# jesusdpa1/ssqueeze_rs

Hardware: NVIDIA B200
Metric: ssq_stft input Msamples/s (higher is better)
Workload: dtype f32

## Files before the change

ssqueeze_rs_b200/csrc/fft_regs.cuh:

```cuda
#pragma once
#include "stft_kernels.cuh"

template <bool PK = true>
__device__ __forceinline__ void fft8_fwd(float2 (&v)[8]) {
  const float S = 0.70710678118654752440f;
  float2 a0 = caddf<PK>(v[0], v[4]), a4 = csubf<PK>(v[0], v[4]);
  float2 a1 = caddf<PK>(v[1], v[5]), a5 = csubf<PK>(v[1], v[5]);
  float2 a2 = caddf<PK>(v[2], v[6]), a6 = csubf<PK>(v[2], v[6]);
  float2 a3 = caddf<PK>(v[3], v[7]), a7 = csubf<PK>(v[3], v[7]);
  float2 p5 = caddf<PK>(a5, cmi(a5));
  float2 p6 = cmi(a6);
  float2 p7 = csubf<PK>(cmi(a7), a7);
  float2 b0 = caddf<PK>(a0, a2), b2 = csubf<PK>(a0, a2);
  float2 b1 = caddf<PK>(a1, a3), b3 = csubf<PK>(a1, a3);
  float2 b4 = caddf<PK>(a4, p6), b6 = csubf<PK>(a4, p6);
  float2 b5 = caddf<PK>(p5, p7), b7 = csubf<PK>(p5, p7);
  float2 r3 = cmi(b3);
  float2 r7 = cmi(b7);
  v[0] = caddf<PK>(b0, b1);
  v[4] = csubf<PK>(b0, b1);
  v[2] = caddf<PK>(b2, r3);
  v[6] = csubf<PK>(b2, r3);
  v[1] = fma2<PK>(b5, bc2(S), b4);
  v[5] = fma2<PK>(b5, bc2(-S), b4);
  v[3] = fma2<PK>(r7, bc2(S), b6);
  v[7] = fma2<PK>(r7, bc2(-S), b6);
}

template <bool PK = true>
__device__ __forceinline__ void fft8_inv(float2 (&v)[8]) {
  const float S = 0.70710678118654752440f;
  float2 a0 = caddf<PK>(v[0], v[4]), a4 = csubf<PK>(v[0], v[4]);
  float2 a1 = caddf<PK>(v[1], v[5]), a5 = csubf<PK>(v[1], v[5]);
  float2 a2 = caddf<PK>(v[2], v[6]), a6 = csubf<PK>(v[2], v[6]);
  float2 a3 = caddf<PK>(v[3], v[7]), a7 = csubf<PK>(v[3], v[7]);
  float2 p5 = caddf<PK>(a5, cpi(a5));
  float2 p6 = cpi(a6);
  float2 p7 = csubf<PK>(cpi(a7), a7);
  float2 b0 = caddf<PK>(a0, a2), b2 = csubf<PK>(a0, a2);
  float2 b1 = caddf<PK>(a1, a3), b3 = csubf<PK>(a1, a3);
  float2 b4 = caddf<PK>(a4, p6), b6 = csubf<PK>(a4, p6);
  float2 b5 = caddf<PK>(p5, p7), b7 = csubf<PK>(p5, p7);
  float2 r3 = cpi(b3);
  float2 r7 = cpi(b7);
  v[0] = caddf<PK>(b0, b1);
  v[4] = csubf<PK>(b0, b1);
  v[2] = caddf<PK>(b2, r3);
  v[6] = csubf<PK>(b2, r3);
  v[1] = fma2<PK>(b5, bc2(S), b4);
  v[5] = fma2<PK>(b5, bc2(-S), b4);
  v[3] = fma2<PK>(r7, bc2(S), b6);
  v[7] = fma2<PK>(r7, bc2(-S), b6);
}

__device__ __forceinline__ float rcp_approx(float x) {
  float r;
  asm("rcp.approx.ftz.f32 %0, %1;" : "=f"(r) : "f"(x));
  return r;
}

__device__ __forceinline__ void smem_rmw_add(float2* p, float re, float im) {
  float2 t = *p;
  t.x += re;
  t.y += im;
  *p = t;
}

struct H32Lane {
  int lane, j2, f1, rd1a, rd1b, g2, wr2;
  float lane_f, j2_f;
  bool l0;
  const float2* tw2;
  float2 tw3a[7], tw3b[7];
};

template <bool ROT = false, bool TW2POW = ROT, bool PK = true>
__device__ __forceinline__ void h32_fft512(const H32Lane& L, float2* xch, float2 (&va)[8], float2 (&vb)[8]) {
  const int lane = L.lane, j2 = L.j2;
  fft8_fwd<PK>(va);
  fft8_fwd<PK>(vb);
  {
    float4* rowa = reinterpret_cast<float4*>(xch + lane * 8);
    float4* rowb = reinterpret_cast<float4*>(xch + (lane + 32) * 8);
#pragma unroll
    for (int q = 0; q < 4; ++q) {
      rowa[q ^ L.f1] = make_float4(va[2 * q].x, va[2 * q].y, va[2 * q + 1].x, va[2 * q + 1].y);
      rowb[q ^ L.f1] = make_float4(vb[2 * q].x, vb[2 * q].y, vb[2 * q + 1].x, vb[2 * q + 1].y);
    }
  }
  __syncwarp();
#pragma unroll
  for (int t = 0; t < 8; ++t) {
    va[t] = xch[L.rd1a + 64 * t];
    vb[t] = xch[L.rd1b + 64 * t];
  }
  __syncwarp();
  {
    float2 w[8];
    w[1] = L.tw2[1];
    if (TW2POW) {
      w[2] = cmulf<PK>(w[1], w[1]);
      w[3] = cmulf<PK>(w[2], w[1]);
      w[4] = cmulf<PK>(w[2], w[2]);
      w[5] = cmulf<PK>(w[4], w[1]);
      w[6] = cmulf<PK>(w[4], w[2]);
      w[7] = cmulf<PK>(w[4], w[3]);
    } else {
#pragma unroll
      for (int t = 2; t < 8; ++t) w[t] = L.tw2[t];
    }
#pragma unroll
    for (int t = 1; t < 8; ++t) {
      va[t] = cmulf<PK>(va[t], w[t]);
      vb[t] = cmulf<PK>(vb[t], w[t]);
    }
  }
  fft8_fwd<PK>(va);
  fft8_fwd<PK>(vb);
#pragma unroll
  for (int t = 0; t < 8; ++t) {
    xch[L.wr2 + 8 * (t ^ L.g2)] = va[t];
    xch[L.wr2 + 256 + 8 * (t ^ L.g2)] = vb[t];
  }
  __syncwarp();
#pragma unroll
  for (int t = 0; t < 8; ++t) {
    va[t] = xch[(lane ^ (8 * (t & 1))) + 64 * t];
    vb[t] = xch[(j2 ^ (8 * (t & 1))) + 64 * t];
  }
  __syncwarp();
  if (ROT) {
    const float C1 = 0.92387953251128673848f, S1 = 0.38268343236508978178f, H = 0.70710678118654752440f;
    const float2 w16[7] = {{C1, -S1}, {H, -H}, {S1, -C1}, {0.f, -1.f}, {-S1, -C1}, {-H, -H}, {-C1, -S1}};
    float2 w3[7];
    w3[0] = L.tw3a[0];
    w3[1] = cmulf<PK>(w3[0], w3[0]);
    w3[2] = cmulf<PK>(w3[1], w3[0]);
    w3[3] = cmulf<PK>(w3[1], w3[1]);
    w3[4] = cmulf<PK>(w3[3], w3[0]);
    w3[5] = cmulf<PK>(w3[3], w3[1]);
    w3[6] = cmulf<PK>(w3[3], w3[2]);
#pragma unroll
    for (int t = 1; t < 8; ++t) {
      const float2 wa = w3[t - 1];
      va[t] = cmulf<PK>(va[t], wa);
      const float2 wb = L.l0 ? w16[t - 1] : wa;
      vb[t] = cmulcf<PK>(vb[t], wb);
    }
    fft8_fwd<PK>(va);
    fft8_inv<PK>(vb);
    return;
  }
#pragma unroll
  for (int t = 1; t < 8; ++t) {
    va[t] = cmulf<PK>(va[t], L.tw3a[t - 1]);
    vb[t] = cmulf<PK>(vb[t], L.tw3b[t - 1]);
  }
  fft8_fwd<PK>(va);
  fft8_fwd<PK>(vb);
}
```

ssqueeze_rs_b200/csrc/stft_h32r.cuh:

```cuda
#pragma once
#include "fft_regs.cuh"

#ifndef H32R_PK
#define H32R_PK(MODE) true
#endif
#define H32R_AS 261

__device__ __forceinline__ int h32r_phys(int k) { return k + (k >> 6); }

struct H32RItem {
  int kb;
  float vre, vim;
};

template <int MODE, int SQZ, bool DBG = false>
__device__ __forceinline__ H32RItem h32r_item(const StftParams& P, float txs, float2* col, float2* colB, float skf,
                                              float2 A, float2 B, size_t dbg_base = 0) {
  H32RItem it;
  const unsigned sgn = __float_as_uint(skf) & 0x80000000u;
  const float2 cd = add2<MODE == 0>(A, make_float2(B.x, -B.y));
  const float c = cd.x, d0 = cd.y;
  if (MODE == 1) {
    const int k = (int)fabsf(skf);
    col[h32r_phys(k)] = make_float2(0.5f * c, __uint_as_float(__float_as_uint(0.5f * d0) ^ sgn));
    if (colB) {
      const float2 ba = add2<MODE == 0>(B, make_float2(-A.x, A.y));
      const float b0 = ba.x, a = ba.y;
      colB[h32r_phys(k)] = make_float2(0.5f * a, __uint_as_float(__float_as_uint(0.5f * b0) ^ sgn));
    }
    it.kb = -1;
    it.vre = it.vim = 0.f;
    return it;
  }
  const float2 ba = add2<MODE == 0>(B, make_float2(-A.x, A.y));
  const float b0 = ba.x, a = ba.y;
  const float den = fmaf(c, c, d0 * d0);
  const float num0 = fmaf(b0, c, -a * d0);
  const float q0 = num0 * rcp_approx(den);
  const float binf = fabsf(fmaf(-q0, P.cphase, skf));
  it.kb = min(max(__float2int_ru(binf - 0.5f), 0), 256);
  if (DBG) {
    const float ms = (txs < 0.f) != (P.tx_scale < 0.f) ? -1.f : 1.f;
    ssq_dbg_emit(P, dbg_base, (int)fabsf(skf), ms * c, ms * __uint_as_float(__float_as_uint(d0) ^ sgn), ms * a,
                 ms * __uint_as_float(__float_as_uint(b0) ^ sgn), binf, den < P.gate2, it.kb);
  }
  if (den < P.gate2) it.kb = -1;
  if (SQZ == SSQ_SQUEEZE_LEBESGUE) {
    it.vre = P.leb_val;
    it.vim = 0.f;
  } else {
    it.vre = c * txs;
    it.vim = d0 * __uint_as_float(__float_as_uint(txs) ^ sgn);
  }
  return it;
}

__device__ __noinline__ void h32r_collision(float2* col, unsigned* T, int kb, float vre, float vim, bool mine,
                                            int lane) {
  const bool on = kb >= 0;
  {
    const unsigned act = __ballot_sync(0xffffffffu, on);
    const int first = __ffs(act) - 1;
    const int kb0 = __shfl_sync(0xffffffffu, kb, first);
    if (__all_sync(0xffffffffu, !on || kb == kb0)) {
      float sr = on ? vre : 0.f, si = on ? vim : 0.f;
#pragma unroll
      for (int o = 16; o > 0; o >>= 1) {
        sr += __shfl_xor_sync(0xffffffffu, sr, o);
        si += __shfl_xor_sync(0xffffffffu, si, o);
      }
      if (lane == first) smem_rmw_add(col + h32r_phys(kb0), sr, si);
      return;
    }
  }
  if (on && !mine) T[kb] = 0xFF;
  __syncwarp();
  const bool contended = on && T[kb] == 0xFF;
  if (on && !contended) smem_rmw_add(col + h32r_phys(kb), vre, vim);
  unsigned m = __ballot_sync(0xffffffffu, contended);
  if (__popc(m) > 4) {
    while (m) {
      const int first = __ffs(m) - 1;
      const int kb0 = __shfl_sync(0xffffffffu, kb, first);
      const bool member = contended && kb == kb0;
      float sr = member ? vre : 0.f, si = member ? vim : 0.f;
#pragma unroll
      for (int o = 16; o > 0; o >>= 1) {
        sr += __shfl_xor_sync(0xffffffffu, sr, o);
        si += __shfl_xor_sync(0xffffffffu, si, o);
      }
      if (lane == first) smem_rmw_add(col + h32r_phys(kb0), sr, si);
      m &= ~__ballot_sync(0xffffffffu, member);
    }
    __syncwarp();
    return;
  }
  while (m) {
    const int src = __ffs(m) - 1;
    m &= m - 1;
    if (lane == src) smem_rmw_add(col + h32r_phys(kb), vre, vim);
    __syncwarp();
  }
}

template <int MODE, int SQZ, bool DBG = false>
__device__ __forceinline__ void h32r_frame(const StftParams& P, const H32Lane& L, float skf0, float wrapd, float txs,
                                           float2* xch, float2* col, float2* colB, float2 (&va)[8], float2 (&vb)[8],
                                           size_t dbg_base = 0) {
  const int lane = L.lane;
  const bool l0 = L.l0;
  unsigned* tagA = reinterpret_cast<unsigned*>(xch);
  unsigned* tagB = tagA + 264;
  h32_fft512<true, true, H32R_PK(MODE)>(L, xch, va, vb);
  __syncwarp();

#define H32R_PAIR(r, A, B)                                   \
  float2 A = va[r], B = vb[r];                               \
  if (l0) {                                                  \
    A = (r) < 4 ? va[r] : vb[(11 - (r)) & 7];                \
    B = (r) < 4 ? va[(8 - (r)) & 7] : vb[((r)-4) & 7];       \
  }

  H32RItem cur;
  float skf = skf0;
  {
    H32R_PAIR(0, A, B)
    cur = h32r_item<MODE, SQZ, DBG>(P, txs, col, colB, skf, A, B, dbg_base);
  }
  if (MODE == 0) {
    if (cur.kb >= 0) tagA[cur.kb] = (unsigned)lane;
    __syncwarp();
  }
#pragma unroll
  for (int r = 0; r < 8; ++r) {
    H32RItem nxt;
    nxt.kb = -1;
    nxt.vre = nxt.vim = 0.f;
    if (r < 7) {
      skf += (skf >= 192.f) ? wrapd : 64.f;
      H32R_PAIR(r + 1, A, B)
      nxt = h32r_item<MODE, SQZ, DBG>(P, txs, col, colB, skf, A, B, dbg_base);
    }
    if (MODE == 0) {
      unsigned* T = (r & 1) ? tagB : tagA;
      unsigned* Tn = (r & 1) ? tagA : tagB;
      const bool on = cur.kb >= 0;
      float2* slot = col + h32r_phys(on ? cur.kb : 0);
      float2 t = *slot;
      const bool mine = !on || T[cur.kb] == (unsigned)lane;
      if (__all_sync(0xffffffffu, mine)) {
        if (on) {
          t.x += cur.vre;
          t.y += cur.vim;
          *slot = t;
        }
      } else {
        h32r_collision(col, T, cur.kb, cur.vre, cur.vim, mine, lane);
      }
      if (r < 7 && nxt.kb >= 0) Tn[nxt.kb] = (unsigned)lane;
      __syncwarp();
    }
    cur = nxt;
  }
#undef H32R_PAIR
  if (l0) {
    const H32RItem it = h32r_item<MODE, SQZ, DBG>(P, txs, col, colB, 256.f, va[4], va[4], dbg_base);
    if (MODE == 0 && it.kb >= 0) smem_rmw_add(col + h32r_phys(it.kb), it.vre, it.vim);
  }
  __syncwarp();
}

__device__ __noinline__ float h32r_edge_sample(const float* x, int64_t n, int64_t p, int left, int padtype,
                                               int64_t origin) {
  return stft_sample<false>(x, n, p, left, padtype, origin);
}

#define H32R_NW(MODE) ((MODE) == 1 ? 8 : 4)


__device__ __forceinline__ void h32r_tmem_st32(uint32_t taddr, const float (&v)[32]) {
  asm volatile(
      "tcgen05.st.sync.aligned.32x32b.x32.b32 [%0], {%1,%2,%3,%4,%5,%6,%7,%8,%9,%10,%11,%12,%13,%14,%15,%16,%17,%18,%19,"
      "%20,%21,%22,%23,%24,%25,%26,%27,%28,%29,%30,%31,%32};\n\t"
      "tcgen05.wait::st.sync.aligned;" ::"r"(taddr),
      "f"(v[0]), "f"(v[1]), "f"(v[2]), "f"(v[3]), "f"(v[4]), "f"(v[5]), "f"(v[6]), "f"(v[7]), "f"(v[8]), "f"(v[9]),
      "f"(v[10]), "f"(v[11]), "f"(v[12]), "f"(v[13]), "f"(v[14]), "f"(v[15]), "f"(v[16]), "f"(v[17]), "f"(v[18]),
      "f"(v[19]), "f"(v[20]), "f"(v[21]), "f"(v[22]), "f"(v[23]), "f"(v[24]), "f"(v[25]), "f"(v[26]), "f"(v[27]),
      "f"(v[28]), "f"(v[29]), "f"(v[30]), "f"(v[31]));
}

__device__ __forceinline__ void h32r_tmem_st16(uint32_t taddr, const float (&v)[17]) {
  asm volatile(
      "tcgen05.st.sync.aligned.32x32b.x16.b32 [%0], {%1,%2,%3,%4,%5,%6,%7,%8,%9,%10,%11,%12,%13,%14,%15,%16};" ::"r"(taddr),
      "f"(v[0]), "f"(v[1]), "f"(v[2]), "f"(v[3]), "f"(v[4]), "f"(v[5]), "f"(v[6]), "f"(v[7]), "f"(v[8]), "f"(v[9]),
      "f"(v[10]), "f"(v[11]), "f"(v[12]), "f"(v[13]), "f"(v[14]), "f"(v[15]));
}

__device__ __forceinline__ void h32r_tmem_st1(uint32_t taddr, float v) {
  asm volatile("tcgen05.st.sync.aligned.32x32b.x1.b32 [%0], {%1};" ::"r"(taddr), "f"(v));
}

__device__ __forceinline__ void h32r_tmem_ld_window(uint32_t taddr_x, uint32_t taddr_w, float (&x)[16], float (&v)[32]) {
  asm volatile(
      "tcgen05.wait::st.sync.aligned;\n\t"
      "tcgen05.ld.sync.aligned.32x32b.x16.b32 {%0,%1,%2,%3,%4,%5,%6,%7,%8,%9,%10,%11,%12,%13,%14,%15}, [%48];\n\t"
      "tcgen05.ld.sync.aligned.32x32b.x32.b32 {%16,%17,%18,%19,%20,%21,%22,%23,%24,%25,%26,%27,%28,%29,%30,%31,%32,%33,"
      "%34,%35,%36,%37,%38,%39,%40,%41,%42,%43,%44,%45,%46,%47}, [%49];\n\t"
      "tcgen05.wait::ld.sync.aligned;"
      : "=f"(x[0]), "=f"(x[1]), "=f"(x[2]), "=f"(x[3]), "=f"(x[4]), "=f"(x[5]), "=f"(x[6]), "=f"(x[7]), "=f"(x[8]),
        "=f"(x[9]), "=f"(x[10]), "=f"(x[11]), "=f"(x[12]), "=f"(x[13]), "=f"(x[14]), "=f"(x[15]),
        "=f"(v[0]), "=f"(v[1]), "=f"(v[2]), "=f"(v[3]), "=f"(v[4]), "=f"(v[5]), "=f"(v[6]), "=f"(v[7]), "=f"(v[8]),
        "=f"(v[9]), "=f"(v[10]), "=f"(v[11]), "=f"(v[12]), "=f"(v[13]), "=f"(v[14]), "=f"(v[15]), "=f"(v[16]),
        "=f"(v[17]), "=f"(v[18]), "=f"(v[19]), "=f"(v[20]), "=f"(v[21]), "=f"(v[22]), "=f"(v[23]), "=f"(v[24]),
        "=f"(v[25]), "=f"(v[26]), "=f"(v[27]), "=f"(v[28]), "=f"(v[29]), "=f"(v[30]), "=f"(v[31])
      : "r"(taddr_x), "r"(taddr_w));
}

__device__ __forceinline__ void h32r_tmem_ld32(uint32_t taddr, float (&v)[32]) {
  asm volatile(
      "tcgen05.ld.sync.aligned.32x32b.x32.b32 {%0,%1,%2,%3,%4,%5,%6,%7,%8,%9,%10,%11,%12,%13,%14,%15,%16,%17,%18,%19,"
      "%20,%21,%22,%23,%24,%25,%26,%27,%28,%29,%30,%31}, [%32];\n\t"
      "tcgen05.wait::ld.sync.aligned;"
      : "=f"(v[0]), "=f"(v[1]), "=f"(v[2]), "=f"(v[3]), "=f"(v[4]), "=f"(v[5]), "=f"(v[6]), "=f"(v[7]), "=f"(v[8]),
        "=f"(v[9]), "=f"(v[10]), "=f"(v[11]), "=f"(v[12]), "=f"(v[13]), "=f"(v[14]), "=f"(v[15]), "=f"(v[16]),
        "=f"(v[17]), "=f"(v[18]), "=f"(v[19]), "=f"(v[20]), "=f"(v[21]), "=f"(v[22]), "=f"(v[23]), "=f"(v[24]),
        "=f"(v[25]), "=f"(v[26]), "=f"(v[27]), "=f"(v[28]), "=f"(v[29]), "=f"(v[30]), "=f"(v[31])
      : "r"(taddr));
}

template <int MODE, int SQZ, bool SLIDE, bool DBG = false>
__global__ void __launch_bounds__(H32R_NW(MODE) * 32, 16 / H32R_NW(MODE)) ssq_stft512_h32r_kernel(const StftParams P) {
  constexpr int N = 512, AS = H32R_AS, NW = H32R_NW(MODE), F = 4 * NW;
  constexpr bool PAIR = (MODE == 1) && SLIDE;
  constexpr bool TM = MODE == 0;
  constexpr bool RING = TM && SLIDE;
  constexpr int TMC = RING ? 64 : 32;
  constexpr int WT = TM ? 0 : N;
  extern __shared__ float2 smem[];
  __shared__ uint32_t tmem_base_s;
  float2* wtab = smem;
  float2* tw2tab = smem + WT;
  float2* acc = smem + WT + 72;
  const int lane = threadIdx.x & 31, warp = threadIdx.x >> 5;
  float2* xch = acc + F * AS + warp * N;

  if (TM && warp == 0) {
    asm volatile("tcgen05.alloc.cta_group::1.sync.aligned.shared::cta.b32 [%0], %1;" ::"r"(
                     (uint32_t)__cvta_generic_to_shared(&tmem_base_s)),
                 "n"(TMC));
    asm volatile("tcgen05.relinquish_alloc_permit.cta_group::1.sync.aligned;");
  }
  if (!TM)
    for (int i = threadIdx.x; i < N; i += blockDim.x) wtab[i] = make_float2(P.win[i], P.dwin[i]);
  if (threadIdx.x < 64)
    tw2tab[(threadIdx.x >> 3) * 9 + (threadIdx.x & 7)] = P.tw[((threadIdx.x >> 3) * (threadIdx.x & 7) * 8) & (N - 1)];
  for (int i = threadIdx.x; i < F * AS; i += blockDim.x) acc[i] = make_float2(0.f, 0.f);

  H32Lane L;
  L.lane = lane;
  L.j2 = lane ? 64 - lane : 32;
  L.tw2 = tw2tab + (lane & 7) * 9;
  const int rho = lane & 7;
  const int ea = lane + 64 * rho;
#pragma unroll
  for (int t = 1; t < 8; ++t) {
    L.tw3a[t - 1] = P.tw[(ea * t) & (N - 1)];
    L.tw3b[t - 1] = make_float2(0.f, 0.f);
  }
  L.f1 = (lane >> 1) & 3;
  L.rd1a = (lane >> 3) * 8 + ((((lane & 7) >> 1) ^ ((lane >> 4) & 3)) << 1) + (lane & 1);
  L.rd1b = ((lane >> 3) + 4) * 8 + ((((lane & 7) >> 1) ^ (((lane >> 4) + 2) & 3)) << 1) + (lane & 1);
  L.g2 = (lane >> 3) & 1;
  L.wr2 = (lane >> 3) * 64 + (lane & 7);
  L.lane_f = (float)lane;
  L.j2_f = (float)L.j2;
  L.l0 = (lane == 0);
  const float txs = (P.modulated && (lane & 1)) ? -P.tx_scale : P.tx_scale;
  float skf0, wrapd;
  if (lane == 0) {
    skf0 = 0.f;
    wrapd = -160.f;
  } else {
    const int ka = lane + 64 * rho;
    skf0 = rho <= 3 ? (float)ka : (float)(ka - 512);
    wrapd = -448.f;
  }
  if (TM) asm volatile("tcgen05.fence::before_thread_sync;");
  __syncthreads();
  uint32_t taps = 0;
  if (TM) {
    asm volatile("tcgen05.fence::after_thread_sync;");
    taps = tmem_base_s + ((uint32_t)(warp * 32) << 16);
    float v[32];
#pragma unroll
    for (int t = 0; t < 8; ++t) {
      v[4 * t] = P.win[lane + 64 * t];
      v[4 * t + 1] = P.dwin[lane + 64 * t];
      v[4 * t + 2] = P.win[lane + 32 + 64 * t];
      v[4 * t + 3] = P.dwin[lane + 32 + 64 * t];
    }
    h32r_tmem_st32(taps, v);
  }

  const float* xc = nullptr;
  int64_t f0 = 0;
  int nfr = 0;
  bool inner = false;
  float xw[17];
  const int64_t lo = P.left + P.x_origin;
  const int tpc = (int)P.tiles_per_channel, ntiles = (int)P.total_tiles;
  auto open_tile = [&](int tile) {
    const int ch = tile / tpc;
    f0 = (int64_t)(tile - ch * tpc) * F + 4 * warp;
    nfr = (int)max((int64_t)0, min((int64_t)4, P.n_frames - f0));
    f0 += P.frame0;
    xc = P.x + (size_t)ch * P.x_stride;
    const int64_t hop = SLIDE ? 32 : P.hop;
    inner = f0 * hop - P.left >= 0 && (f0 + 3) * hop + N - 1 - P.left + (PAIR ? 32 : 0) < P.n;
    if (nfr > 0) {
      const int64_t p = f0 * hop + lane;
      if (inner) {
#pragma unroll
        for (int j = 0; j < (PAIR ? 17 : 16); ++j) xw[j] = __ldg(xc + (p + 32 * j - lo));
      } else {
#pragma unroll
        for (int j = 0; j < (PAIR ? 17 : 16); ++j) xw[j] = h32r_edge_sample(xc, P.n, p + 32 * j, P.left, P.padtype, P.x_origin);
      }
    }
  };

  for (int tile = (int)blockIdx.x - (int)gridDim.x; tile < ntiles; tile += (int)gridDim.x) {
    const bool real = tile >= 0;
    const int tch = real ? tile / tpc : 0;
    const int64_t tf0 = real ? (int64_t)(tile - tch * tpc) * F : 0;
    const int tnf = real ? (int)min((int64_t)F, P.n_frames - tf0) : 0;
    const int next = tile + (int)gridDim.x;
    const int my_n = real ? nfr : 0;
    if (RING && real) h32r_tmem_st16(taps + 32, xw);
#pragma unroll 1
    for (int s = 0; s < 4; s += (PAIR ? 2 : 1)) {
      const bool active = s < my_n;
      float2 va[8], vb[8];
      float xn = 0.f;
      if (active) {
        float tv[TM ? 32 : 1];
        float xs[RING ? 16 : 1];
        if constexpr (RING)
          h32r_tmem_ld_window(taps + 32 + s, taps, xs, tv);
        else if constexpr (TM)
          h32r_tmem_ld32(taps, tv);
#pragma unroll
        for (int t = 0; t < 8; ++t) {
          float2 w0, w1;
          if constexpr (TM) {
            w0 = make_float2(tv[4 * t], tv[4 * t + 1]);
            w1 = make_float2(tv[4 * t + 2], tv[4 * t + 3]);
          } else {
            w0 = wtab[lane + 64 * t];
            w1 = wtab[lane + 32 + 64 * t];
          }
          if (PAIR) {
            va[t] = mul2<false>(make_float2(xw[2 * t], xw[2 * t + 1]), bc2(w0.x));
            vb[t] = mul2<false>(make_float2(xw[2 * t + 1], xw[2 * t + 2]), bc2(w1.x));
          } else if constexpr (RING) {
            va[t] = mul2(bc2(xs[2 * t]), w0);
            vb[t] = mul2(bc2(xs[2 * t + 1]), w1);
          } else {
            va[t] = mul2(bc2(xw[2 * t]), w0);
            vb[t] = mul2(bc2(xw[2 * t + 1]), w1);
          }
        }
      }
      if (s == (PAIR ? 2 : 3)) {
        if (!RING && next < ntiles) open_tile(next);
      } else if (s + (PAIR ? 2 : 1) < my_n) {
        if (PAIR) {
#pragma unroll
          for (int j = 0; j < 15; ++j) xw[j] = xw[j + 2];
          const int64_t p = (f0 + s + 2) * 32 + lane + 480;
          if (inner) {
            xw[15] = __ldg(xc + (p - lo));
            xw[16] = __ldg(xc + (p + 32 - lo));
          } else {
            xw[15] = h32r_edge_sample(xc, P.n, p, P.left, P.padtype, P.x_origin);
            xw[16] = h32r_edge_sample(xc, P.n, p + 32, P.left, P.padtype, P.x_origin);
          }
        } else if (RING) {
          const int64_t p = (f0 + s + 1) * 32 + lane + 480;
          xn = inner ? __ldg(xc + (p - lo)) : h32r_edge_sample(xc, P.n, p, P.left, P.padtype, P.x_origin);
        } else if (SLIDE) {
#pragma unroll
          for (int j = 0; j < 15; ++j) xw[j] = xw[j + 1];
          const int64_t p = (f0 + s + 1) * 32 + lane + 480;
          xw[15] = inner ? __ldg(xc + (p - lo)) : h32r_edge_sample(xc, P.n, p, P.left, P.padtype, P.x_origin);
        } else {
          const int64_t p = (f0 + s + 1) * (int64_t)P.hop + lane;
          if (inner) {
#pragma unroll
            for (int j = 0; j < 16; ++j) xw[j] = __ldg(xc + (p + 32 * j - lo));
          } else {
#pragma unroll
            for (int j = 0; j < 16; ++j) xw[j] = h32r_edge_sample(xc, P.n, p + 32 * j, P.left, P.padtype, P.x_origin);
          }
        }
      }
      if (active)
        h32r_frame<MODE, SQZ, DBG>(P, L, skf0, wrapd, txs, xch, acc + (4 * warp + s) * AS,
                                   PAIR ? acc + (4 * warp + s + 1) * AS : nullptr, va, vb,
                                   DBG ? (size_t)tch * 257 * P.n_frames + tf0 + 4 * warp + s : 0);
      if (RING && s + 1 < my_n) h32r_tmem_st1(taps + 48 + s, xn);
    }
    if (RING && next < ntiles) open_tile(next);
    if (!real) continue;
    __syncthreads();
    {
      const int fr = threadIdx.x % F, v = threadIdx.x / F;
      float2* a = acc + fr * AS + v;
      float2* g = P.out + ((size_t)tch * 257 + v) * P.n_frames + tf0 + fr;
      const size_t gstep = (size_t)8 * P.n_frames;
      const bool ok = fr < tnf;
#pragma unroll 1
      for (int io = 0; io < 4; ++io) {
#pragma unroll
        for (int ii = 0; ii < 8; ++ii) {
          const float2 val = a[8 * ii];
          if (MODE == 0) a[8 * ii] = make_float2(0.f, 0.f);
          if (ok) __stcs(g, val);
          g += gstep;
        }
        a += 65;
      }
      if (v == 0) {
        const float2 val = a[0];
        if (MODE == 0) a[0] = make_float2(0.f, 0.f);
        if (ok) __stcs(g, val);
      }
    }
    __syncthreads();
  }
  if (TM) {
    asm volatile("tcgen05.fence::before_thread_sync;");
    __syncthreads();
    asm volatile("tcgen05.fence::after_thread_sync;");
    if (warp == 0)
      asm volatile("tcgen05.dealloc.cta_group::1.sync.aligned.b32 %0, %1;" ::"r"(tmem_base_s), "n"(TMC));
  }
}

static ssq_status stft_h32r_launch(ssq_ctx* ctx, StftParams& P, bool* done) {
  *done = false;
  if (P.n_fft != 512 || ctx->opt.no_h32r) return SSQ_OK;
  const int NW = H32R_NW(P.mode), F = 4 * NW;
  P.F = F;
  P.acc_stride = H32R_AS;
  P.tiles_per_channel = (P.n_frames + F - 1) / F;
  P.total_tiles = P.tiles_per_channel * P.channels;
  if (P.total_tiles > (int64_t)0x7ff00000) return SSQ_OK;
  *done = true;
  const size_t wt = P.mode == 1 ? 512 : 0;
  const size_t smem = (wt + 72 + (size_t)F * H32R_AS + (size_t)NW * 512) * sizeof(float2);
  const int grid = (int)std::min<int64_t>(P.total_tiles, (int64_t)ctx->num_sms * (16 / NW));
  const bool leb = P.squeezing == SSQ_SQUEEZE_LEBESGUE;
  void (*k)(const StftParams);
  const bool dbg = P.mode == 0 && (P.aux_Sx || P.aux_dSx || P.aux_w || P.aux_kb);
  if (dbg)
    k = P.hop == 32 ? (leb ? ssq_stft512_h32r_kernel<0, 1, true, true> : ssq_stft512_h32r_kernel<0, 0, true, true>)
                    : (leb ? ssq_stft512_h32r_kernel<0, 1, false, true> : ssq_stft512_h32r_kernel<0, 0, false, true>);
  else if (P.hop == 32)
    k = P.mode == 1 ? ssq_stft512_h32r_kernel<1, 0, true>
        : leb       ? ssq_stft512_h32r_kernel<0, 1, true>
                    : ssq_stft512_h32r_kernel<0, 0, true>;
  else
    k = P.mode == 1 ? ssq_stft512_h32r_kernel<1, 0, false>
        : leb       ? ssq_stft512_h32r_kernel<0, 1, false>
                    : ssq_stft512_h32r_kernel<0, 0, false>;
  SSQ_CUDA_TRY(ctx, cudaFuncSetAttribute(k, cudaFuncAttributeMaxDynamicSharedMemorySize, (int)smem));
  k<<<grid, NW * 32, smem, ctx->stream>>>(P);
  const char* name = P.mode == 1 ? "ssq_stft512_h32r_kernel<stft>" : "ssq_stft512_h32r_kernel<ssq>";
  SSQ_TRY(ssq_check_launch(ctx, name));
  ctx->last_kernel = name;
  return SSQ_OK;
}
```

Baseline: 22530.

## Route FFT512 transposes through tensor memory instead of shared memory in SSQ mode

In the synchrosqueezing path (MODE 0), the two warp-level data exchanges of the 512-point register FFT now go through Blackwell tensor memory via tcgen05 st/ld with different shapes, plus a shuffle, in place of the swizzled shared-memory writes and reads. Lanes are permuted (sigma) so window taps, input samples and twiddle rows match the new data layout, and the TMEM allocation doubles to hold the exchange columns. Per-warp shared scratch shrinks and the epilogue recomputes tile indices to save registers. The aim is less shared-memory traffic and fewer bank conflicts in the FFT transposes, at the cost of added TMEM wait latency and more layout complexity.

```diff
diff --git a/ssqueeze_rs_b200/csrc/fft_regs.cuh b/ssqueeze_rs_b200/csrc/fft_regs.cuh
--- a/ssqueeze_rs_b200/csrc/fft_regs.cuh
+++ b/ssqueeze_rs_b200/csrc/fft_regs.cuh
@@ -74,6 +74,53 @@
   float2 tw3a[7], tw3b[7];
 };
 
+template <bool TW2POW, bool PK>
+__device__ __forceinline__ void h32_stage2(const H32Lane& L, float2 (&va)[8], float2 (&vb)[8]) {
+  float2 w[8];
+  w[1] = L.tw2[1];
+  if (TW2POW) {
+    w[2] = cmulf<PK>(w[1], w[1]);
+    w[3] = cmulf<PK>(w[2], w[1]);
+    w[4] = cmulf<PK>(w[2], w[2]);
+    w[5] = cmulf<PK>(w[4], w[1]);
+    w[6] = cmulf<PK>(w[4], w[2]);
+    w[7] = cmulf<PK>(w[4], w[3]);
+  } else {
+#pragma unroll
+    for (int t = 2; t < 8; ++t) w[t] = L.tw2[t];
+  }
+#pragma unroll
+  for (int t = 1; t < 8; ++t) {
+    va[t] = cmulf<PK>(va[t], w[t]);
+    vb[t] = cmulf<PK>(vb[t], w[t]);
+  }
+  fft8_fwd<PK>(va);
+  fft8_fwd<PK>(vb);
+}
+
+template <bool PK>
+__device__ __forceinline__ void h32_stage3_rot(const H32Lane& L, float2 (&va)[8], float2 (&vb)[8]) {
+  const float C1 = 0.92387953251128673848f, S1 = 0.38268343236508978178f, H = 0.70710678118654752440f;
+  const float2 w16[7] = {{C1, -S1}, {H, -H}, {S1, -C1}, {0.f, -1.f}, {-S1, -C1}, {-H, -H}, {-C1, -S1}};
+  float2 w3[7];
+  w3[0] = L.tw3a[0];
+  w3[1] = cmulf<PK>(w3[0], w3[0]);
+  w3[2] = cmulf<PK>(w3[1], w3[0]);
+  w3[3] = cmulf<PK>(w3[1], w3[1]);
+  w3[4] = cmulf<PK>(w3[3], w3[0]);
+  w3[5] = cmulf<PK>(w3[3], w3[1]);
+  w3[6] = cmulf<PK>(w3[3], w3[2]);
+#pragma unroll
+  for (int t = 1; t < 8; ++t) {
+    const float2 wa = w3[t - 1];
+    va[t] = cmulf<PK>(va[t], wa);
+    const float2 wb = L.l0 ? w16[t - 1] : wa;
+    vb[t] = cmulcf<PK>(vb[t], wb);
+  }
+  fft8_fwd<PK>(va);
+  fft8_inv<PK>(vb);
+}
+
 template <bool ROT = false, bool TW2POW = ROT, bool PK = true>
 __device__ __forceinline__ void h32_fft512(const H32Lane& L, float2* xch, float2 (&va)[8], float2 (&vb)[8]) {
   const int lane = L.lane, j2 = L.j2;
@@ -95,28 +142,7 @@
     vb[t] = xch[L.rd1b + 64 * t];
   }
   __syncwarp();
-  {
-    float2 w[8];
-    w[1] = L.tw2[1];
-    if (TW2POW) {
-      w[2] = cmulf<PK>(w[1], w[1]);
-      w[3] = cmulf<PK>(w[2], w[1]);
-      w[4] = cmulf<PK>(w[2], w[2]);
-      w[5] = cmulf<PK>(w[4], w[1]);
-      w[6] = cmulf<PK>(w[4], w[2]);
-      w[7] = cmulf<PK>(w[4], w[3]);
-    } else {
-#pragma unroll
-      for (int t = 2; t < 8; ++t) w[t] = L.tw2[t];
-    }
-#pragma unroll
-    for (int t = 1; t < 8; ++t) {
-      va[t] = cmulf<PK>(va[t], w[t]);
-      vb[t] = cmulf<PK>(vb[t], w[t]);
-    }
-  }
-  fft8_fwd<PK>(va);
-  fft8_fwd<PK>(vb);
+  h32_stage2<TW2POW, PK>(L, va, vb);
 #pragma unroll
   for (int t = 0; t < 8; ++t) {
     xch[L.wr2 + 8 * (t ^ L.g2)] = va[t];
@@ -130,25 +156,7 @@
   }
   __syncwarp();
   if (ROT) {
-    const float C1 = 0.92387953251128673848f, S1 = 0.38268343236508978178f, H = 0.70710678118654752440f;
-    const float2 w16[7] = {{C1, -S1}, {H, -H}, {S1, -C1}, {0.f, -1.f}, {-S1, -C1}, {-H, -H}, {-C1, -S1}};
-    float2 w3[7];
-    w3[0] = L.tw3a[0];
-    w3[1] = cmulf<PK>(w3[0], w3[0]);
-    w3[2] = cmulf<PK>(w3[1], w3[0]);
-    w3[3] = cmulf<PK>(w3[1], w3[1]);
-    w3[4] = cmulf<PK>(w3[3], w3[0]);
-    w3[5] = cmulf<PK>(w3[3], w3[1]);
-    w3[6] = cmulf<PK>(w3[3], w3[2]);
-#pragma unroll
-    for (int t = 1; t < 8; ++t) {
-      const float2 wa = w3[t - 1];
-      va[t] = cmulf<PK>(va[t], wa);
-      const float2 wb = L.l0 ? w16[t - 1] : wa;
-      vb[t] = cmulcf<PK>(vb[t], wb);
-    }
-    fft8_fwd<PK>(va);
-    fft8_inv<PK>(vb);
+    h32_stage3_rot<PK>(L, va, vb);
     return;
   }
 #pragma unroll
diff --git a/ssqueeze_rs_b200/csrc/stft_h32r.cuh b/ssqueeze_rs_b200/csrc/stft_h32r.cuh
--- a/ssqueeze_rs_b200/csrc/stft_h32r.cuh
+++ b/ssqueeze_rs_b200/csrc/stft_h32r.cuh
@@ -103,16 +103,99 @@
   }
 }
 
-template <int MODE, int SQZ, bool DBG = false>
+template <int C>
+__device__ __forceinline__ void h32r_tm_xch_z(uint32_t taddr, float (&v)[32]) {
+  asm volatile(
+      "tcgen05.st.sync.aligned.32x32b.x32.b32 [%32+%33], {%0,%1,%2,%3,%4,%5,%6,%7,%8,%9,%10,%11,%12,%13,%14,%15,"
+      "%16,%17,%18,%19,%20,%21,%22,%23,%24,%25,%26,%27,%28,%29,%30,%31};\n\t"
+      "tcgen05.wait::st.sync.aligned;\n\t"
+      "tcgen05.ld.sync.aligned.16x32bx2.x8.b32 {%0,%1,%2,%3,%4,%5,%6,%7}, [%32+%33], 16;\n\t"
+      "tcgen05.ld.sync.aligned.16x32bx2.x8.b32 {%8,%9,%10,%11,%12,%13,%14,%15}, [%32+%34], 16;\n\t"
+      "tcgen05.ld.sync.aligned.16x32bx2.x8.b32 {%16,%17,%18,%19,%20,%21,%22,%23}, [%32+%36], 16;\n\t"
+      "tcgen05.ld.sync.aligned.16x32bx2.x8.b32 {%24,%25,%26,%27,%28,%29,%30,%31}, [%32+%37], 16;\n\t"
+      "tcgen05.wait::ld.sync.aligned;"
+      : "+f"(v[0]), "+f"(v[1]), "+f"(v[2]), "+f"(v[3]), "+f"(v[4]), "+f"(v[5]), "+f"(v[6]), "+f"(v[7]), "+f"(v[8]),
+        "+f"(v[9]), "+f"(v[10]), "+f"(v[11]), "+f"(v[12]), "+f"(v[13]), "+f"(v[14]), "+f"(v[15]), "+f"(v[16]),
+        "+f"(v[17]), "+f"(v[18]), "+f"(v[19]), "+f"(v[20]), "+f"(v[21]), "+f"(v[22]), "+f"(v[23]), "+f"(v[24]),
+        "+f"(v[25]), "+f"(v[26]), "+f"(v[27]), "+f"(v[28]), "+f"(v[29]), "+f"(v[30]), "+f"(v[31])
+      : "r"(taddr), "n"(C), "n"(C + 8), "n"(C + 16), "n"(C + (16 << 16)), "n"(C + 8 + (16 << 16)),
+        "n"(C + 16 + (16 << 16)));
+}
+
+template <int C>
+__device__ __forceinline__ void h32r_tm_xch_y(uint32_t taddr, float (&v)[32]) {
+  asm volatile(
+      "tcgen05.st.sync.aligned.16x256b.x2.b32 [%32+%33], {%0,%1,%2,%3,%4,%5,%6,%7};\n\t"
+      "tcgen05.st.sync.aligned.16x256b.x2.b32 [%32+%36], {%8,%9,%10,%11,%12,%13,%14,%15};\n\t"
+      "tcgen05.st.sync.aligned.16x256b.x2.b32 [%32+%35], {%16,%17,%18,%19,%20,%21,%22,%23};\n\t"
+      "tcgen05.st.sync.aligned.16x256b.x2.b32 [%32+%38], {%24,%25,%26,%27,%28,%29,%30,%31};\n\t"
+      "tcgen05.wait::st.sync.aligned;\n\t"
+      "tcgen05.ld.sync.aligned.32x32b.x16.b32 {%0,%1,%2,%3,%4,%5,%6,%7,%8,%9,%10,%11,%12,%13,%14,%15}, [%32+%33];\n\t"
+      "tcgen05.ld.sync.aligned.32x32b.x16.b32 {%16,%17,%18,%19,%20,%21,%22,%23,%24,%25,%26,%27,%28,%29,%30,%31}, [%32+%35];\n\t"
+      "tcgen05.wait::ld.sync.aligned;"
+      : "+f"(v[0]), "+f"(v[1]), "+f"(v[2]), "+f"(v[3]), "+f"(v[4]), "+f"(v[5]), "+f"(v[6]), "+f"(v[7]), "+f"(v[8]),
+        "+f"(v[9]), "+f"(v[10]), "+f"(v[11]), "+f"(v[12]), "+f"(v[13]), "+f"(v[14]), "+f"(v[15]), "+f"(v[16]),
+        "+f"(v[17]), "+f"(v[18]), "+f"(v[19]), "+f"(v[20]), "+f"(v[21]), "+f"(v[22]), "+f"(v[23]), "+f"(v[24]),
+        "+f"(v[25]), "+f"(v[26]), "+f"(v[27]), "+f"(v[28]), "+f"(v[29]), "+f"(v[30]), "+f"(v[31])
+      : "r"(taddr), "n"(C), "n"(C + 8), "n"(C + 16), "n"(C + (16 << 16)), "n"(C + 8 + (16 << 16)),
+        "n"(C + 16 + (16 << 16)));
+}
+
+__device__ __forceinline__ int h32r_sigma(int lane) { return (lane >> 2) | ((lane & 3) << 3); }
+
+template <int XC, bool PK>
+__device__ __forceinline__ void h32r_fft512_tm(const H32Lane& L, uint32_t taps, float2 (&va)[8], float2 (&vb)[8]) {
+  fft8_fwd<PK>(va);
+  fft8_fwd<PK>(vb);
+  float u[32];
+#pragma unroll
+  for (int k = 0; k < 8; ++k) {
+    const int i = 2 * (((k >> 1) & 1) + 4 * (k >> 2) + 8 * (k & 1));
+    u[i] = va[k].x;
+    u[i + 1] = va[k].y;
+    u[i + 4] = vb[k].x;
+    u[i + 5] = vb[k].y;
+  }
+  h32r_tm_xch_z<XC>(taps, u);
+  h32r_tm_xch_y<XC>(taps, u);
+#pragma unroll
+  for (int t = 0; t < 8; ++t) {
+    va[t] = make_float2(u[2 * t], u[2 * t + 1]);
+    vb[t] = make_float2(u[16 + 2 * t], u[17 + 2 * t]);
+  }
+  h32_stage2<true, PK>(L, va, vb);
+#pragma unroll
+  for (int k = 0; k < 8; ++k) {
+    const int i = 8 * (2 * (k >> 2) + ((k >> 1) & 1)) + 2 * (k & 1);
+    u[i] = va[k].x;
+    u[i + 1] = va[k].y;
+    u[i + 4] = vb[k].x;
+    u[i + 5] = vb[k].y;
+  }
+  h32r_tm_xch_y<XC>(taps, u);
+  const int src = (32 - L.lane) & 31;
+#pragma unroll
+  for (int t = 0; t < 8; ++t) {
+    va[t] = make_float2(u[2 * t], u[2 * t + 1]);
+    vb[t] = make_float2(__shfl_sync(0xffffffffu, u[16 + 2 * t], src), __shfl_sync(0xffffffffu, u[17 + 2 * t], src));
+  }
+  h32_stage3_rot<PK>(L, va, vb);
+}
+
+template <int MODE, int SQZ, int XC, bool DBG = false>
 __device__ __forceinline__ void h32r_frame(const StftParams& P, const H32Lane& L, float skf0, float wrapd, float txs,
-                                           float2* xch, float2* col, float2* colB, float2 (&va)[8], float2 (&vb)[8],
-                                           size_t dbg_base = 0) {
+                                           float2* xch, uint32_t taps, float2* col, float2* colB, float2 (&va)[8],
+                                           float2 (&vb)[8], size_t dbg_base = 0) {
   const int lane = L.lane;
   const bool l0 = L.l0;
   unsigned* tagA = reinterpret_cast<unsigned*>(xch);
   unsigned* tagB = tagA + 264;
-  h32_fft512<true, true, H32R_PK(MODE)>(L, xch, va, vb);
-  __syncwarp();
+  if constexpr (MODE == 0) {
+    h32r_fft512_tm<XC, H32R_PK(MODE)>(L, taps, va, vb);
+  } else {
+    h32_fft512<true, true, H32R_PK(MODE)>(L, xch, va, vb);
+    __syncwarp();
+  }
 
 #define H32R_PAIR(r, A, B)                                   \
   float2 A = va[r], B = vb[r];                               \
@@ -234,7 +317,8 @@
   constexpr bool PAIR = (MODE == 1) && SLIDE;
   constexpr bool TM = MODE == 0;
   constexpr bool RING = TM && SLIDE;
-  constexpr int TMC = RING ? 64 : 32;
+  constexpr int TMC = RING ? 128 : 64;
+  constexpr int XC = RING ? 64 : 32;
   constexpr int WT = TM ? 0 : N;
   extern __shared__ float2 smem[];
   __shared__ uint32_t tmem_base_s;
@@ -242,7 +326,7 @@
   float2* tw2tab = smem + WT;
   float2* acc = smem + WT + 72;
   const int lane = threadIdx.x & 31, warp = threadIdx.x >> 5;
-  float2* xch = acc + F * AS + warp * N;
+  float2* xch = acc + F * AS + warp * (TM ? 264 : N);
 
   if (TM && warp == 0) {
     asm volatile("tcgen05.alloc.cta_group::1.sync.aligned.shared::cta.b32 [%0], %1;" ::"r"(
@@ -259,7 +343,7 @@
   H32Lane L;
   L.lane = lane;
   L.j2 = lane ? 64 - lane : 32;
-  L.tw2 = tw2tab + (lane & 7) * 9;
+  L.tw2 = tw2tab + (TM ? lane >> 2 : lane & 7) * 9;
   const int rho = lane & 7;
   const int ea = lane + 64 * rho;
 #pragma unroll
@@ -288,22 +372,23 @@
   if (TM) asm volatile("tcgen05.fence::before_thread_sync;");
   __syncthreads();
   uint32_t taps = 0;
+  const int sl = TM ? h32r_sigma(lane) : lane;
   if (TM) {
     asm volatile("tcgen05.fence::after_thread_sync;");
     taps = tmem_base_s + ((uint32_t)(warp * 32) << 16);
     float v[32];
 #pragma unroll
     for (int t = 0; t < 8; ++t) {
-      v[4 * t] = P.win[lane + 64 * t];
-      v[4 * t + 1] = P.dwin[lane + 64 * t];
-      v[4 * t + 2] = P.win[lane + 32 + 64 * t];
-      v[4 * t + 3] = P.dwin[lane + 32 + 64 * t];
+      v[4 * t] = P.win[sl + 64 * t];
+      v[4 * t + 1] = P.dwin[sl + 64 * t];
+      v[4 * t + 2] = P.win[sl + 32 + 64 * t];
+      v[4 * t + 3] = P.dwin[sl + 32 + 64 * t];
     }
     h32r_tmem_st32(taps, v);
   }
 
   const float* xc = nullptr;
-  int64_t f0 = 0;
+  int64_t p0 = 0;
   int nfr = 0;
   bool inner = false;
   float xw[17];
@@ -311,29 +396,26 @@
   const int tpc = (int)P.tiles_per_channel, ntiles = (int)P.total_tiles;
   auto open_tile = [&](int tile) {
     const int ch = tile / tpc;
-    f0 = (int64_t)(tile - ch * tpc) * F + 4 * warp;
+    int64_t f0 = (int64_t)(tile - ch * tpc) * F + 4 * warp;
     nfr = (int)max((int64_t)0, min((int64_t)4, P.n_frames - f0));
     f0 += P.frame0;
     xc = P.x + (size_t)ch * P.x_stride;
     const int64_t hop = SLIDE ? 32 : P.hop;
     inner = f0 * hop - P.left >= 0 && (f0 + 3) * hop + N - 1 - P.left + (PAIR ? 32 : 0) < P.n;
+    p0 = f0 * hop + sl;
     if (nfr > 0) {
-      const int64_t p = f0 * hop + lane;
       if (inner) {
 #pragma unroll
-        for (int j = 0; j < (PAIR ? 17 : 16); ++j) xw[j] = __ldg(xc + (p + 32 * j - lo));
+        for (int j = 0; j < (PAIR ? 17 : 16); ++j) xw[j] = __ldg(xc + (p0 + 32 * j - lo));
       } else {
 #pragma unroll
-        for (int j = 0; j < (PAIR ? 17 : 16); ++j) xw[j] = h32r_edge_sample(xc, P.n, p + 32 * j, P.left, P.padtype, P.x_origin);
+        for (int j = 0; j < (PAIR ? 17 : 16); ++j) xw[j] = h32r_edge_sample(xc, P.n, p0 + 32 * j, P.left, P.padtype, P.x_origin);
       }
     }
   };
 
   for (int tile = (int)blockIdx.x - (int)gridDim.x; tile < ntiles; tile += (int)gridDim.x) {
     const bool real = tile >= 0;
-    const int tch = real ? tile / tpc : 0;
-    const int64_t tf0 = real ? (int64_t)(tile - tch * tpc) * F : 0;
-    const int tnf = real ? (int)min((int64_t)F, P.n_frames - tf0) : 0;
     const int next = tile + (int)gridDim.x;
     const int my_n = real ? nfr : 0;
     if (RING && real) h32r_tmem_st16(taps + 32, xw);
@@ -377,7 +459,7 @@
         if (PAIR) {
 #pragma unroll
           for (int j = 0; j < 15; ++j) xw[j] = xw[j + 2];
-          const int64_t p = (f0 + s + 2) * 32 + lane + 480;
+          const int64_t p = p0 + (s + 2) * 32 + 480;
           if (inner) {
             xw[15] = __ldg(xc + (p - lo));
             xw[16] = __ldg(xc + (p + 32 - lo));
@@ -386,15 +468,15 @@
             xw[16] = h32r_edge_sample(xc, P.n, p + 32, P.left, P.padtype, P.x_origin);
           }
         } else if (RING) {
-          const int64_t p = (f0 + s + 1) * 32 + lane + 480;
+          const int64_t p = p0 + (s + 1) * 32 + 480;
           xn = inner ? __ldg(xc + (p - lo)) : h32r_edge_sample(xc, P.n, p, P.left, P.padtype, P.x_origin);
         } else if (SLIDE) {
 #pragma unroll
           for (int j = 0; j < 15; ++j) xw[j] = xw[j + 1];
-          const int64_t p = (f0 + s + 1) * 32 + lane + 480;
+          const int64_t p = p0 + (s + 1) * 32 + 480;
           xw[15] = inner ? __ldg(xc + (p - lo)) : h32r_edge_sample(xc, P.n, p, P.left, P.padtype, P.x_origin);
         } else {
-          const int64_t p = (f0 + s + 1) * (int64_t)P.hop + lane;
+          const int64_t p = p0 + (s + 1) * (int64_t)P.hop;
           if (inner) {
 #pragma unroll
             for (int j = 0; j < 16; ++j) xw[j] = __ldg(xc + (p + 32 * j - lo));
@@ -405,20 +487,27 @@
         }
       }
       if (active)
-        h32r_frame<MODE, SQZ, DBG>(P, L, skf0, wrapd, txs, xch, acc + (4 * warp + s) * AS,
+        h32r_frame<MODE, SQZ, XC, DBG>(P, L, skf0, wrapd, txs, xch, taps, acc + (4 * warp + s) * AS,
                                    PAIR ? acc + (4 * warp + s + 1) * AS : nullptr, va, vb,
-                                   DBG ? (size_t)tch * 257 * P.n_frames + tf0 + 4 * warp + s : 0);
+                                   DBG ? (size_t)(tile / tpc) * 257 * P.n_frames + (tile % tpc) * (int64_t)F + 4 * warp + s : 0);
       if (RING && s + 1 < my_n) h32r_tmem_st1(taps + 48 + s, xn);
     }
     if (RING && next < ntiles) open_tile(next);
-    if (!real) continue;
+    unsigned nct;
+    asm volatile("mov.u32 %0, %%nctaid.x;" : "=r"(nct));
+    const int cur = next - (int)nct;
+    if (cur < 0) continue;
     __syncthreads();
     {
-      const int fr = threadIdx.x % F, v = threadIdx.x / F;
+      unsigned tid;
+      asm volatile("mov.u32 %0, %%tid.x;" : "=r"(tid));
+      const int fr = tid % F, v = tid / F;
+      const int tch = cur / tpc;
+      const int64_t tf0 = (int64_t)(cur - tch * tpc) * F;
       float2* a = acc + fr * AS + v;
       float2* g = P.out + ((size_t)tch * 257 + v) * P.n_frames + tf0 + fr;
       const size_t gstep = (size_t)8 * P.n_frames;
-      const bool ok = fr < tnf;
+      const bool ok = fr < P.n_frames - tf0;
 #pragma unroll 1
       for (int io = 0; io < 4; ++io) {
 #pragma unroll
@@ -457,8 +546,8 @@
   P.total_tiles = P.tiles_per_channel * P.channels;
   if (P.total_tiles > (int64_t)0x7ff00000) return SSQ_OK;
   *done = true;
-  const size_t wt = P.mode == 1 ? 512 : 0;
-  const size_t smem = (wt + 72 + (size_t)F * H32R_AS + (size_t)NW * 512) * sizeof(float2);
+  const size_t wt = P.mode == 1 ? 512 : 0, xs = P.mode == 1 ? 512 : 264;
+  const size_t smem = (wt + 72 + (size_t)F * H32R_AS + (size_t)NW * xs) * sizeof(float2);
   const int grid = (int)std::min<int64_t>(P.total_tiles, (int64_t)ctx->num_sms * (16 / NW));
   const bool leb = P.squeezing == SSQ_SQUEEZE_LEBESGUE;
   void (*k)(const StftParams);
```

Result: faster. 23820, median of 6 (+5.7%).
